# NVlabs/FoundationPose

Hardware: NVIDIA H100
Metric: pose-hypotheses/sec at 640x480 RGB-D, 252 hyp, 5 refine iters (higher is better)
Workload: dtype f16

## Files before the change

foundationpose_b200/csrc/fp_api.cu:

```cuda
#include <math.h>
#include <stdlib.h>
#include <string.h>

#include <algorithm>
#include <exception>
#include <map>
#include <memory>
#include <string>
#include <tuple>
#include <utility>
#include <vector>

#include "../../include/fpose.h"
#include "fp_attn.cuh"
#include "fp_common.cuh"
#include "fp_crop.cuh"
#include "fp_depth.cuh"
#include "fp_gemm.cuh"
#include "fp_vis.cuh"

namespace fp {
const char* get_last_error();

template <cudaError_t (*Free)(void*)>
// ... 74 lines not shown
struct MeshSlot {
  DevBuf vpos, vnrm, vatt, faces, meshlets, ml_verts, ml_tris, tex;
  int V = 0, F = 0, Ht = 0, Wt = 0, n_meshlets = 0, front_sign = 0, closed = 0;
  float bs[4] = {0.f, 0.f, 0.f, 0.f};
  bool has_tex = false, loaded = false;
  float diameter = 0.f;
};

struct CameraBufs {
  DevBuf rgb_raw, depth_raw, rgba, depth, xyz;
  PinnedBuf stage_rgb, stage_depth;
};

}

struct fp_ctx {
  int device = 0;
  fp::Net net[2];
  unsigned long long epoch = 1;
  unsigned long long graph_captures = 0;
  fp::MeshSlot mesh[fp::kMaxMeshes];
  fp::DevBuf mesh_table;
  float rot_normalizer = 0.3490658503988659f;
  float crop_ratio[2] = {1.2f, 1.2f};
  fp::CameraBufs cam[fp::kMaxCameras];
  fp::DevBuf depth_a;
  const float* depth_cur = nullptr;
  float K[9] = {0};
  int H = 0, W = 0;
  bool has_frame = false;
  int cap_n = 0;
  fp::DevBuf crops, act0, a1, a2, a3, ab0, ab1, ab2, c0, c1, c2, tok, qkv, att, x1pre, x1, ff, x2pre;
  fp::DevBuf head_out, poses_a, poses_b, feats, tail_qkv, tail_attn, tail_proj, scores, best;
  int tail_cap = 0;
  float fold_c = 0.f;
  fp::DevBuf fold_v, tail_counter;
  struct GraphEntry {
    cudaGraphExec_t exec = nullptr;
    unsigned long long epoch = 0;
    float K[9] = {0};
    int H = 0, W = 0;
  };
  std::map<std::tuple<int, int, int, int>, GraphEntry> graphs;
  std::map<std::tuple<int, int, int, int>, int> graph_nodes;
  cudaStream_t cap_stream = nullptr;
  cudaStream_t side_stream = nullptr;
  cudaEvent_t ev_fork = nullptr, ev_join = nullptr;
  int fork_max_n = 128;
  bool use_graphs = true;
  bool cull_backfaces = true;
  bool track_valid = false;
  int crop_tile = 0;
  fp::DevBuf lt_buf, lr_buf, feat_buf, pose_stage, tok_mean;
  fp::DevBuf mask_buf, mask_stats, crop_stats;
  fp::PinnedBuf stage_pose;
  fp::DevBuf track_pose;
  fp::PinnedBuf stage_poses;
  fp::DevBuf args;
  fp::PinnedBuf stage_args;
  int cam_grid_h = 0, cam_grid_w = 0;
  fp::DevBuf seg_off, reg_feats, mask_off;
  fp::PinnedBuf stage_masks, stage_ints;
  fp::DevBuf vis_rec, vis_range;
};

namespace fp {

static int ensure_capacity(fp_ctx* c, int N) {
  if (N <= c->cap_n) return 0;
  const size_t n = (size_t)N;
  int rc = 0;
  const size_t m = 2 * n + 3;
  rc |= dev_alloc(c->epoch, c->crops, m * kCropImg * 2, true);
  rc |= dev_alloc(c->epoch, c->act0, m * 80 * 80 * 64 * 2);
  rc |= dev_alloc(c->epoch, c->a1, m * 1600 * 128 * 2);
  rc |= dev_alloc(c->epoch, c->a2, m * 1600 * 128 * 2);
  rc |= dev_alloc(c->epoch, c->a3, m * 1600 * 128 * 2);
  rc |= dev_alloc(c->epoch, c->ab0, n * 1600 * 256 * 2);
  rc |= dev_alloc(c->epoch, c->ab1, n * 1600 * 256 * 2);
  rc |= dev_alloc(c->epoch, c->ab2, n * 1600 * 256 * 2);
  rc |= dev_alloc(c->epoch, c->c0, n * T * 512 * 2);
  rc |= dev_alloc(c->epoch, c->c1, n * T * 512 * 2);
  rc |= dev_alloc(c->epoch, c->c2, n * T * 512 * 2);
  rc |= dev_alloc(c->epoch, c->tok, n * T * 512 * 2);
  rc |= dev_alloc(c->epoch, c->qkv, n * T * 3072 * 2);
  rc |= dev_alloc(c->epoch, c->att, 2 * n * T * 512 * 2);
  rc |= dev_alloc(c->epoch, c->x1pre, 2 * n * T * 512 * 2);
  rc |= dev_alloc(c->epoch, c->x1, 2 * n * T * 512 * 2);
  rc |= dev_alloc(c->epoch, c->ff, 2 * n * T * 512 * 2);
  rc |= dev_alloc(c->epoch, c->x2pre, 2 * n * T * 512 * 2);
  rc |= dev_alloc(c->epoch, c->head_out, 2 * n * 3 * 4);
  rc |= dev_alloc(c->epoch, c->poses_a, n * 16 * 4);
  rc |= dev_alloc(c->epoch, c->poses_b, n * 16 * 4);
  rc |= dev_alloc(c->epoch, c->feats, n * 512 * 4);
  rc |= dev_alloc(c->epoch, c->lt_buf, n * 3 * 4);
  rc |= dev_alloc(c->epoch, c->lr_buf, n * 9 * 4);
  rc |= dev_alloc(c->epoch, c->feat_buf, n * 512 * 4);
  rc |= dev_alloc(c->epoch, c->pose_stage, n * 16 * 4);
  rc |= dev_alloc(c->epoch, c->tok_mean, n * 512 * 4);
  if (rc) return -2;
  c->cap_n = N;
  return 0;
}

static int ensure_tail(fp_ctx* c, int L) {
  if (L <= c->tail_cap) return 0;
  int rc = 0;
  rc |= dev_alloc(c->epoch, c->tail_qkv, (size_t)L * 1536 * 4);
  rc |= dev_alloc(c->epoch, c->tail_attn, (size_t)L * 512 * 4);
  rc |= dev_alloc(c->epoch, c->tail_proj, (size_t)L * 512 * 4);
  rc |= dev_alloc(c->epoch, c->scores, (size_t)L * 4);
  rc |= dev_alloc(c->epoch, c->best, 16);
  if (rc) return -2;
  c->tail_cap = L;
  return 0;
}

static GemmLayer mk(int kind, int n_img, int H, int W, int Cin, int Cout, const void* in, const __half* w,
                    const float* b, void* out, int relu, const void* res = nullptr, int out_ld = 0, int out_split = 0,
                    const float* post_add = nullptr) {
  GemmLayer L;
  L.kind = kind;
  L.n_img = n_img;
  L.Hin = H;
// ... 33 lines not shown
  FP_TRY(gemm_layer_launch(mk(LK_CONV3_S1, M, 40, 40, 128, 128, c->a2.p, W(5), B(5), c->ab0.p, 1, c->a3.p, 256, Np), st));
  FP_TRY(gemm_layer_launch(mk(LK_CONV3_S1, N, 40, 40, 256, 256, c->ab0.p, W(6), B(6), c->ab1.p, 1), st));
  FP_TRY(gemm_layer_launch(mk(LK_CONV3_S1, N, 40, 40, 256, 256, c->ab1.p, W(7), B(7), c->ab2.p, 1, c->ab0.p), st));
  FP_TRY(gemm_layer_launch(mk(LK_CONV3_S1, N, 40, 40, 256, 256, c->ab2.p, W(8), B(8), c->ab1.p, 1), st));
  FP_TRY(gemm_layer_launch(mk(LK_CONV3_S1, N, 40, 40, 256, 256, c->ab1.p, W(9), B(9), c->ab0.p, 1, c->ab2.p), st));
  FP_TRY(gemm_layer_launch(mk(LK_CONV3_S2, N, 40, 40, 256, 512, c->ab0.p, W(10), B(10), c->c0.p, 1), st));
  FP_TRY(gemm_layer_launch(mk(LK_CONV3_S1, N, 20, 20, 512, 512, c->c0.p, W(11), B(11), c->c1.p, 1), st));
  FP_TRY(gemm_layer_launch(mk(LK_CONV3_S1, N, 20, 20, 512, 512, c->c1.p, W(12), B(12), c->c2.p, 1, c->c0.p), st));
  FP_TRY(gemm_layer_launch(mk(LK_CONV3_S1, N, 20, 20, 512, 512, c->c2.p, W(13), B(13), c->c1.p, 1), st));
  FP_TRY(gemm_layer_launch(
      mk(LK_CONV3_S1, N, 20, 20, 512, 512, c->c1.p, W(14), B(14), c->tok.p, 1, c->c2.p, 0, 0, net.f("pe")), st));
  return 0;
}

static int run_refine_heads(fp_ctx* c, const Net& net, int N, cudaStream_t st) {
  const int M = N * T;
  FP_TRY(gemm_layer_launch(mk(LK_LINEAR, 1, 1, M, 512, 3072, c->tok.p, net.h("heads.in_w"), net.f("heads.in_b"), c->qkv.p, 0), st));
  AttnParams ap;
  ap.qkv = reinterpret_cast<const __half*>(c->qkv.p);
  ap.ld = 3072;
  ap.q_off = 0;
  ap.k_off = 512;
  ap.v_off = 1024;
  ap.group_col_stride = 1536;
  ap.n_groups = 2;
  ap.out = reinterpret_cast<__half*>(c->att.p);
  ap.ld_out = 512;
  ap.out_group_stride = (size_t)M * 512;
  ap.B = N;
  ap.T = T;
  ap.n_heads = 4;
  ap.scale = 0.08838834764831845f;
  FP_TRY(attn_core_launch(ap, st));
  const bool fork = N <= c->fork_max_n;
  if (fork) {
    if (!c->side_stream) {
      FP_CUDA_OK(cudaStreamCreateWithFlags(&c->side_stream, cudaStreamNonBlocking));
      FP_CUDA_OK(cudaEventCreateWithFlags(&c->ev_fork, cudaEventDisableTiming));
      FP_CUDA_OK(cudaEventCreateWithFlags(&c->ev_join, cudaEventDisableTiming));
    }
    FP_CUDA_OK(cudaEventRecord(c->ev_fork, st));
    FP_CUDA_OK(cudaStreamWaitEvent(c->side_stream, c->ev_fork, 0));
  }
  for (int g = 0; g < 2; ++g) {
    cudaStream_t sg = (fork && g == 1) ? c->side_stream : st;
    char nm[48];
    auto H = [&](const char* s) { snprintf(nm, sizeof nm, "head%d.%s", g, s); return net.h(nm); };
    auto Fp = [&](const char* s) { snprintf(nm, sizeof nm, "head%d.%s", g, s); return net.f(nm); };
    const size_t off = (size_t)g * M * 512;
    const __half* att_g = reinterpret_cast<const __half*>(c->att.p) + off;
    __half* x1pre = reinterpret_cast<__half*>(c->x1pre.p) + off;
    __half* x1 = reinterpret_cast<__half*>(c->x1.p) + off;
    __half* ff = reinterpret_cast<__half*>(c->ff.p) + off;
    __half* x2pre = reinterpret_cast<__half*>(c->x2pre.p) + off;
    const __half* w;
    const float* b;
    w = H("out_w"); b = Fp("out_b");
    if (fork && g == 1) pdl_skip_next();
    FP_TRY(gemm_layer_launch(mk(LK_LINEAR, 1, 1, M, 512, 512, att_g, w, b, x1pre, 0, c->tok.p), sg));
    const float* g1 = Fp("ln1_g");
    const float* b1 = Fp("ln1_b");
    FP_TRY(layernorm_launch(x1pre, x1, g1, b1, M, sg));
    w = H("ff1_w"); b = Fp("ff1_b");
    FP_TRY(gemm_layer_launch(mk(LK_LINEAR, 1, 1, M, 512, 512, x1, w, b, ff, 1), sg));
    w = H("ff2_w"); b = Fp("ff2_b");
    FP_TRY(gemm_layer_launch(mk(LK_LINEAR, 1, 1, M, 512, 512, ff, w, b, x2pre, 0, x1), sg));
    const float* g2 = Fp("ln2_g");
    const float* b2 = Fp("ln2_b");
    const float* fw = Fp("fin_w");
    const float* fb = Fp("fin_b");
    FP_TRY(head_final_launch(x2pre, g2, b2, fw, fb, reinterpret_cast<float*>(c->head_out.p) + (size_t)g * N * 3, N, T, 3, sg));
  }
  if (fork) {
    FP_CUDA_OK(cudaEventRecord(c->ev_join, c->side_stream));
    FP_CUDA_OK(cudaStreamWaitEvent(st, c->ev_join, 0));
    pdl_skip_next();
  }
  return 0;
}

static int run_score_feats(fp_ctx* c, const Net& net, int N, float* feats, cudaStream_t st) {
  const int M = N * T;
  FP_TRY(gemm_layer_launch(mk(LK_LINEAR, 1, 1, M, 512, 1536, c->tok.p, net.h("att.in_w"), net.f("att.in_b"), c->qkv.p, 0), st));
  AttnParams ap;
  ap.qkv = reinterpret_cast<const __half*>(c->qkv.p);
  ap.ld = 1536;
  ap.q_off = 0;
  ap.k_off = 512;
  ap.v_off = 1024;
  ap.group_col_stride = 0;
  ap.n_groups = 1;
// ... 515 lines not shown
#define FP_API_BEGIN try {
#define FP_API_END                                                        \
  }                                                                       \
  catch (const std::exception& e) {                                       \
    fp::set_last_error("%s: exception: %s", __func__, e.what());          \
    return -3;                                                            \
  }                                                                       \
  catch (...) {                                                           \
    fp::set_last_error("%s: unknown exception", __func__);                \
    return -3;                                                            \
  }

extern "C" {

int fp_create(fp_ctx** out) {
  FP_API_BEGIN
  if (!out) {
    set_last_error("fp_create: null output");
    return -1;
  }
  int dev = 0;
  FP_CUDA_OK(cudaGetDevice(&dev));
  cudaDeviceProp prop;
  FP_CUDA_OK(cudaGetDeviceProperties(&prop, dev));
  FP_REQUIRE(prop.major == 9 && prop.minor == 0, "libfpose targets sm_90a (H100); device %d is sm_%d%d", dev, prop.major,
             prop.minor);
  fp_ctx* c = new fp_ctx();
  c->device = dev;
  const char* ng = getenv("FPOSE_NO_GRAPH");
  c->use_graphs = !(ng && ng[0] == '1');
  const char* nc = getenv("FPOSE_NO_CULL");
  c->cull_backfaces = !(nc && nc[0] == '1');
  if (const char* fk = getenv("FPOSE_FORK_MAX_N")) c->fork_max_n = atoi(fk);
  *out = c;
  return 0;
  FP_API_END
}

int fp_destroy(fp_ctx* c) {
  FP_API_BEGIN
  if (!c) return 0;
  DeviceGuard dg(c->device);
  cudaDeviceSynchronize();
  for (auto& kv : c->graphs)
    if (kv.second.exec) cudaGraphExecDestroy(kv.second.exec);
  if (c->cap_stream) cudaStreamDestroy(c->cap_stream);
  if (c->side_stream) cudaStreamDestroy(c->side_stream);
  if (c->ev_fork) cudaEventDestroy(c->ev_fork);
  if (c->ev_join) cudaEventDestroy(c->ev_join);
  delete c;
  return 0;
  FP_API_END
}

int fp_set_config(fp_ctx* c, int which, float crop_ratio, float rot_normalizer) {
  FP_API_BEGIN
  FP_REQUIRE(c, "null ctx");
  FP_REQUIRE(which == 0 || which == 1, "fp_set_config: which must be 0 (refiner) or 1 (scorer)");
  FP_REQUIRE(crop_ratio > 0.f, "fp_set_config: crop_ratio must be positive");
  DeviceGuard dg(c->device);
  c->crop_ratio[which] = crop_ratio;
  if (which == 0) c->rot_normalizer = rot_normalizer;
  ++c->epoch;
  if (c->mesh_table.p) FP_TRY(write_mesh_table(c));
  return 0;
  FP_API_END
// ... 796 lines not shown
```

foundationpose_b200/csrc/fp_api_ops.cu:

```cuda
#include "../../include/fpose.h"
#include "fp_common.cuh"
#include "fp_attn.cuh"
#include "fp_crop.cuh"
#include "fp_gemm.cuh"

#include <vector>

namespace fp {
const char* get_last_error();
int prof_collect(int kind, double* total_ms, double* total_work, int* launches);
int pose_errors_launch(const float* pts, int P, const float* pred, int N, const float* gt, int n_gt, float* add_out,
                       float* adds_out, cudaStream_t stream);
int sym_pose_errors_launch(const float* pts, int P, const float* pred, int N, const float* gt, int n_gt, const float* sym,
                           int S, const float* K, int n_K, float* mssd_out, float* mspd_out, cudaStream_t stream);
}

static int check_device_ptr(const void* p, const char* what, const char* fn = "fp_pose_errors") {
  int dev = 0;
  FP_CUDA_OK(cudaGetDevice(&dev));
  cudaPointerAttributes a;
  const cudaError_t e = cudaPointerGetAttributes(&a, p);
  if (e != cudaSuccess) {
    cudaGetLastError();
    fp::set_last_error("%s: %s: cudaPointerGetAttributes failed (%s)", fn, what, cudaGetErrorString(e));
// ... 82 lines not shown
    info[5] = total;
    return 0;
  } catch (...) {
    fp::set_last_error("fp_op_build_meshlets: exception");
    return -3;
  }
}

int fp_op_attention(const void* qkv, void* out, int B, int impl, void* stream) {
  if (!qkv || !out) {
    fp::set_last_error("fp_op_attention: null argument");
    return -1;
  }
  fp::AttnParams ap;
  ap.qkv = reinterpret_cast<const __half*>(qkv);
  ap.ld = 1536;
  ap.q_off = 0;
  ap.k_off = 512;
  ap.v_off = 1024;
  ap.group_col_stride = 0;
  ap.n_groups = 1;
  ap.out = reinterpret_cast<__half*>(out);
  ap.ld_out = 512;
  ap.out_group_stride = 0;
  ap.B = B;
  ap.T = 400;
  ap.n_heads = 4;
  ap.scale = 0.08838834764831845f;
  cudaStream_t st = reinterpret_cast<cudaStream_t>(stream);
  (void)impl;
  return fp::attn_tc_launch(ap, st);
}

static fp::GemmLayer to_gemm_layer(const fp_gemm_layer_t* l) {
  fp::GemmLayer L;
  L.kind = l->kind;
  L.n_img = l->n_img;
  L.Hin = l->Hin;
  L.Win = l->Win;
  L.Cin = l->Cin;
  L.Cout = l->Cout;
  L.in = l->in;
  L.w = l->w;
  L.bias = l->bias;
  L.res = l->res;
  L.res_ld = l->res_ld;
  L.out = l->out;
  L.out_ld = l->out_ld;
  L.out_split = l->out_split;
  L.post_add = l->post_add;
  L.relu = l->relu;
  return L;
}

int fp_op_gemm_layer(const fp_gemm_layer_t* l, void* stream) {
  if (!l) {
    fp::set_last_error("fp_op_gemm_layer: null layer");
    return -1;
  }
  return fp::gemm_layer_launch(to_gemm_layer(l), reinterpret_cast<cudaStream_t>(stream));
}

int fp_op_gemm_tile_n(const fp_gemm_layer_t* l, int* tile_n) {
  if (!l || !tile_n) {
    fp::set_last_error("fp_op_gemm_tile_n: null argument");
    return -1;
// ... 39 lines not shown
```

foundationpose_b200/csrc/fp_attn.cuh:

```cuda
#pragma once
#include <cuda_fp16.h>
#include <cuda_runtime.h>
#include <stddef.h>

namespace fp {

struct AttnParams {
  const __half* qkv;
  int ld;
  int q_off, k_off, v_off;
  int group_col_stride;
  int n_groups;
  __half* out;
  int ld_out;
  size_t out_group_stride;
  int B, T, n_heads;
  float scale;
};
int attn_core_launch(const AttnParams& p, cudaStream_t stream);
int attn_tc_launch(const AttnParams& p, cudaStream_t stream);

int layernorm_launch(const __half* x, __half* y, const float* gamma, const float* beta, int rows, cudaStream_t stream);
int head_final_launch(const __half* x, const float* gamma, const float* beta, const float* w, const float* bias,
                      float* out, int B, int T, int out_dim, cudaStream_t stream);
int token_mean_proj_launch(const __half* x, const float* w_f32, const float* bias, float* mean_ws, float* out, int B, int T,
                           cudaStream_t stream);

struct ScoreTailParams {
  const float* feats;
  int L;
  const float* w_in;
  const float* b_in;
  const float* fold_v;
  float fold_c;
  float offset;
  float* qkv;
  float* scores;
  int* best;
  unsigned int* counter;
  const int* seg = nullptr;
  int n_seg = 1;
  int seg_max = 0;
};
int score_tail_launch(const ScoreTailParams& p, cudaStream_t stream);

struct MeshSlotDev;
int pose_update_launch(const float* pose_in, const float* trans, const float* rot, float* pose_out,
                       float* trans_delta_out, float* rot_delta_out, int N, const MeshSlotDev* slots, const int* mesh_of,
                       float trans_scale, float rot_normalizer, cudaStream_t stream);
int f32_to_f16_launch(const float* x, __half* y, size_t n, cudaStream_t stream);

}
```

foundationpose_b200/csrc/fp_common.cuh:

```cuda
#pragma once
#include <cuda.h>
#include <cuda_fp16.h>
#include <cuda_runtime.h>
#include <stdint.h>
#include <stdio.h>
#include <string.h>

#include <atomic>

namespace fp {

void note_launches(int n);
unsigned long long launch_count();
void set_capturing(bool on);
inline bool device_bit_test(const std::atomic<unsigned long long>& m) {
  int d = 0;
  cudaGetDevice(&d);
  return (m.load(std::memory_order_acquire) >> (d & 63)) & 1ull;
}
inline void device_bit_set(std::atomic<unsigned long long>& m) {
  int d = 0;
  cudaGetDevice(&d);
  m.fetch_or(1ull << (d & 63), std::memory_order_release);
}
// ... 76 lines not shown
      "mbarrier.try_wait.parity.shared::cta.b64 P1, [%0], %1, %2;\n\t"
      "@P1 bra DONE_%=;\n\t"
      "bra WAIT_%=;\n\t"
      "DONE_%=:\n\t"
      "}" ::"r"(smem_u32(bar)),
      "r"(parity), "r"(0x989680)
      : "memory");
}

__device__ __forceinline__ void tma_load_5d(const CUtensorMap* map, uint64_t* bar, void* dst,
                                            int c0, int c1, int c2, int c3, int c4) {
  asm volatile(
      "cp.async.bulk.tensor.5d.shared::cluster.global.mbarrier::complete_tx::bytes"
      " [%0], [%1, {%3, %4, %5, %6, %7}], [%2];" ::"r"(smem_u32(dst)),
      "l"(reinterpret_cast<uint64_t>(map)), "r"(smem_u32(bar)), "r"(c0), "r"(c1), "r"(c2),
      "r"(c3), "r"(c4)
      : "memory");
}
__device__ __forceinline__ void tma_load_2d(const CUtensorMap* map, uint64_t* bar, void* dst,
                                            int c0, int c1) {
  asm volatile(
      "cp.async.bulk.tensor.2d.shared::cluster.global.mbarrier::complete_tx::bytes"
      " [%0], [%1, {%3, %4}], [%2];" ::"r"(smem_u32(dst)),
      "l"(reinterpret_cast<uint64_t>(map)), "r"(smem_u32(bar)), "r"(c0), "r"(c1)
      : "memory");
}
__device__ __forceinline__ void tma_store_5d(const CUtensorMap* map, const void* src, int c0, int c1, int c2, int c3,
                                             int c4) {
  asm volatile("cp.async.bulk.tensor.5d.global.shared::cta.bulk_group [%0, {%2, %3, %4, %5, %6}], [%1];" ::"l"(
                   reinterpret_cast<uint64_t>(map)),
               "r"(smem_u32(src)), "r"(c0), "r"(c1), "r"(c2), "r"(c3), "r"(c4)
               : "memory");
}
__device__ __forceinline__ void tma_prefetch_desc(const CUtensorMap* map) {
  asm volatile("prefetch.tensormap [%0];" ::"l"(reinterpret_cast<uint64_t>(map)) : "memory");
}

__device__ __forceinline__ uint32_t cluster_nctarank() {
  uint32_t r;
  asm volatile("mov.u32 %0, %%cluster_nctarank;" : "=r"(r));
  return r;
}
__device__ __forceinline__ uint32_t cluster_ctarank() {
  uint32_t r;
  asm volatile("mov.u32 %0, %%cluster_ctarank;" : "=r"(r));
  return r;
}
__device__ __forceinline__ void cluster_sync_all() {
  asm volatile("barrier.cluster.arrive.release.aligned;" ::: "memory");
  asm volatile("barrier.cluster.wait.acquire.aligned;" ::: "memory");
}

template <uint32_t N>
__device__ __forceinline__ void regs_release() {
  asm volatile("setmaxnreg.dec.sync.aligned.u32 %0;" ::"n"(N));
}
template <uint32_t N>
__device__ __forceinline__ void regs_acquire() {
  asm volatile("setmaxnreg.inc.sync.aligned.u32 %0;" ::"n"(N));
}

__device__ __forceinline__ void wgmma_fence() { asm volatile("wgmma.fence.sync.aligned;" ::: "memory"); }
__device__ __forceinline__ void wgmma_commit() { asm volatile("wgmma.commit_group.sync.aligned;" ::: "memory"); }
template <int N>
__device__ __forceinline__ void wgmma_wait() {
  asm volatile("wgmma.wait_group.sync.aligned %0;" ::"n"(N) : "memory");
// ... 38 lines not shown
```

foundationpose_b200/ops.py:

```python
import ctypes as C

import torch

from . import _lib
from ._lib import lib


def _ptr(t):
    return None if t is None else C.c_void_p(t.data_ptr())


def _stream():
    return C.c_void_p(torch.cuda.current_stream().cuda_stream)


def _require_cuda(*ts):
    for t in ts:
        if t is not None and not t.is_cuda:
            raise _lib.FposeError("libfpose operators need CUDA tensors (there is no CPU path)")


def gemm_layer(kind, x, w_packed, bias, *, n_img, Hin, Win, Cin, Cout, out=None, out_ld=None, out_split=0,
               res=None, res_ld=0, post_add=None, relu=False):
    _require_cuda(x, w_packed, bias, res, post_add, out)
# ... 3 lines not shown
    elif kind == _lib.LAYER_CONV3_S1:
        Ho, Wo = Hin, Win
    else:
        Ho, Wo = Hin // 2, Win // 2
    if out is None:
        out_ld = Cout
        out = torch.empty(n_img, Ho, Wo, Cout, dtype=torch.float16, device=x.device)
    L = _lib.GemmLayer(kind, n_img, Hin, Win, Cin, Cout, _ptr(x), _ptr(w_packed), _ptr(bias), _ptr(res),
                       res_ld, _ptr(out), out_ld, out_split, _ptr(post_add), 1 if relu else 0)
    _lib.check(lib.fp_op_gemm_layer(C.byref(L), _stream()), "fp_op_gemm_layer")
    return out


def gemm_tile_n(kind, *, n_img, Hin, Win, Cin, Cout, out_split=0):
    lib.fp_op_gemm_tile_n.argtypes = [C.POINTER(_lib.GemmLayer), C.POINTER(C.c_int)]
    lib.fp_op_gemm_tile_n.restype = C.c_int
    L = _lib.GemmLayer(kind, n_img, Hin, Win, Cin, Cout, None, None, None, None, 0, None, Cout, out_split, None, 0)
    tile_n = C.c_int(0)
    _lib.check(lib.fp_op_gemm_tile_n(C.byref(L), C.byref(tile_n)), "fp_op_gemm_tile_n")
    return tile_n.value


lib.fp_op_attention.argtypes = [C.c_void_p, C.c_void_p, C.c_int, C.c_int, C.c_void_p]
lib.fp_op_attention.restype = C.c_int


def attention(qkv, impl=1):
    _require_cuda(qkv)
    assert qkv.dtype == torch.float16 and qkv.shape[1] == 1536 and qkv.shape[0] % 400 == 0
    B = qkv.shape[0] // 400
    out = torch.empty(qkv.shape[0], 512, dtype=torch.float16, device=qkv.device)
    _lib.check(lib.fp_op_attention(_ptr(qkv), _ptr(out), B, impl, _stream()), "fp_op_attention")
    return out
```

include/fpose.h:

```cpp
#ifndef FPOSE_H_
#define FPOSE_H_

#include <stddef.h>
#include <stdint.h>

#ifdef __cplusplus
extern "C" {
#endif

const char* fp_last_error(void);
unsigned long long fp_launch_count(void);

int fp_prof_enable(int on);
int fp_prof_collect(int kind, double* total_ms, double* total_work, int* launches);


#define FP_LAYER_LINEAR 0
#define FP_LAYER_CONV3_S1 1
#define FP_LAYER_CONV3_S2 2
#define FP_LAYER_CONV7_S2 3

typedef struct fp_gemm_layer {
  int kind;
  int n_img;
  int Hin, Win;
  int Cin;
  int Cout;
  const void* in;
  const void* w;
  const float* bias;
  const void* res;
  int res_ld;
  void* out;
  int out_ld;
  int out_split;
  const float* post_add;
  int relu;
} fp_gemm_layer_t;

int fp_op_gemm_layer(const fp_gemm_layer_t* layer, void* stream);
int fp_op_gemm_tile_n(const fp_gemm_layer_t* layer, int* tile_n);

int fp_op_attention(const void* qkv, void* out, int B, int impl, void* stream);



#define FP_METRICS_MAX_POINTS 131072
#define FP_METRICS_MAX_POSES (1 << 24)
int fp_pose_errors(const float* pts, int P, const float* pred, int N, const float* gt, int n_gt,
                   float* add_out, float* adds_out, void* stream);

#define FP_METRICS_MAX_SYMMETRIES 4096
int fp_sym_pose_errors(const float* pts, int P, const float* pred, int N, const float* gt, int n_gt, const float* sym,
                       int S, const float* K, int n_K, float* mssd_out, float* mspd_out, void* stream);

typedef struct fp_ctx fp_ctx;

int fp_create(fp_ctx** ctx);
int fp_destroy(fp_ctx* ctx);

int fp_set_config(fp_ctx* ctx, int which, float crop_ratio, float rot_normalizer);

typedef struct fp_tensor {
  const char* name;
  const void* data;
  int dtype;
  long long numel;
} fp_tensor_t;

int fp_load_network(fp_ctx* ctx, int which, const fp_tensor_t* tensors, int n);

int fp_set_mesh(fp_ctx* ctx, int V, int F, const float* pos, const float* nrm, const float* uv, const float* vcol,
                const int* faces, const unsigned char* tex_rgb, int Ht, int Wt, float diameter);
#define FP_MAX_MESHES 64
int fp_set_mesh_slot(fp_ctx* ctx, int slot, int V, int F, const float* pos, const float* nrm, const float* uv,
                     const float* vcol, const int* faces, const unsigned char* tex_rgb, int Ht, int Wt, float diameter);
// ... 81 lines not shown
```

Before: 3609.

## Fuse head out-proj/ff2 GEMMs with residual, LayerNorm and readout in full-row kernel

```diff
diff --git a/foundationpose_b200/csrc/fp_api.cu b/foundationpose_b200/csrc/fp_api.cu
--- a/foundationpose_b200/csrc/fp_api.cu
+++ b/foundationpose_b200/csrc/fp_api.cu
@@ -130,6 +130,7 @@
   int cap_n = 0;
   fp::DevBuf crops, act0, a1, a2, a3, ab0, ab1, ab2, c0, c1, c2, tok, qkv, att, x1pre, x1, ff, x2pre;
   fp::DevBuf head_out, poses_a, poses_b, feats, tail_qkv, tail_attn, tail_proj, scores, best;
+  fp::DevBuf head_tok;
   int tail_cap = 0;
   float fold_c = 0.f;
   fp::DevBuf fold_v, tail_counter;
@@ -144,6 +145,7 @@
   cudaStream_t cap_stream = nullptr;
   cudaStream_t side_stream = nullptr;
   cudaEvent_t ev_fork = nullptr, ev_join = nullptr;
+  bool fused_heads = true;
   int fork_max_n = 128;
   bool use_graphs = true;
   bool cull_backfaces = true;
@@ -188,6 +190,7 @@
   rc |= dev_alloc(c->epoch, c->ff, 2 * n * T * 512 * 2);
   rc |= dev_alloc(c->epoch, c->x2pre, 2 * n * T * 512 * 2);
   rc |= dev_alloc(c->epoch, c->head_out, 2 * n * 3 * 4);
+  rc |= dev_alloc(c->epoch, c->head_tok, 2 * n * T * 3 * 4);
   rc |= dev_alloc(c->epoch, c->poses_a, n * 16 * 4);
   rc |= dev_alloc(c->epoch, c->poses_b, n * 16 * 4);
   rc |= dev_alloc(c->epoch, c->feats, n * 512 * 4);
@@ -287,6 +290,7 @@
   ap.n_heads = 4;
   ap.scale = 0.08838834764831845f;
   FP_TRY(attn_core_launch(ap, st));
+  const bool fused = c->fused_heads;
   const bool fork = N <= c->fork_max_n;
   if (fork) {
     if (!c->side_stream) {
@@ -312,6 +316,32 @@
     const float* b;
     w = H("out_w"); b = Fp("out_b");
     if (fork && g == 1) pdl_skip_next();
+    if (fused) {
+      HeadLnArgs a;
+      a.M = M;
+      a.x = att_g;
+      a.w = w;
+      a.bias = b;
+      a.res = reinterpret_cast<const __half*>(c->tok.p);
+      a.gamma = Fp("ln1_g");
+      a.beta = Fp("ln1_b");
+      a.out = x1;
+      a.fin_w = nullptr;
+      a.tok_out = nullptr;
+      FP_TRY(head_ln1_launch(a, sg));
+      FP_TRY(gemm_layer_launch(mk(LK_LINEAR, 1, 1, M, 512, 512, x1, H("ff1_w"), Fp("ff1_b"), ff, 1), sg));
+      a.x = ff;
+      a.w = H("ff2_w");
+      a.bias = Fp("ff2_b");
+      a.res = x1;
+      a.gamma = Fp("ln2_g");
+      a.beta = Fp("ln2_b");
+      a.out = nullptr;
+      a.fin_w = Fp("fin_w");
+      a.tok_out = reinterpret_cast<float*>(c->head_tok.p) + (size_t)g * M * 3;
+      FP_TRY(head_readout_launch(a, Fp("fin_b"), reinterpret_cast<float*>(c->head_out.p) + (size_t)g * N * 3, N, T, sg));
+      continue;
+    }
     FP_TRY(gemm_layer_launch(mk(LK_LINEAR, 1, 1, M, 512, 512, att_g, w, b, x1pre, 0, c->tok.p), sg));
     const float* g1 = Fp("ln1_g");
     const float* b1 = Fp("ln1_b");
@@ -893,6 +923,8 @@
   const char* nc = getenv("FPOSE_NO_CULL");
   c->cull_backfaces = !(nc && nc[0] == '1');
   if (const char* fk = getenv("FPOSE_FORK_MAX_N")) c->fork_max_n = atoi(fk);
+  const char* fh = getenv("FPOSE_FUSED_HEADS");
+  c->fused_heads = !(fh && fh[0] == '0');
   *out = c;
   return 0;
   FP_API_END
diff --git a/foundationpose_b200/csrc/fp_api_ops.cu b/foundationpose_b200/csrc/fp_api_ops.cu
--- a/foundationpose_b200/csrc/fp_api_ops.cu
+++ b/foundationpose_b200/csrc/fp_api_ops.cu
@@ -138,6 +138,53 @@
   return fp::attn_tc_launch(ap, st);
 }
 
+static fp::HeadLnArgs head_args(int M, const void* x, const void* w, const float* bias, const void* res,
+                                const float* gamma, const float* beta) {
+  fp::HeadLnArgs a;
+  a.M = M;
+  a.x = reinterpret_cast<const __half*>(x);
+  a.w = reinterpret_cast<const __half*>(w);
+  a.bias = bias;
+  a.res = reinterpret_cast<const __half*>(res);
+  a.gamma = gamma;
+  a.beta = beta;
+  a.out = nullptr;
+  a.fin_w = nullptr;
+  a.tok_out = nullptr;
+  return a;
+}
+
+int fp_op_head_ln1(int M, const void* x, const void* w, const float* bias, const void* res, const float* gamma,
+                   const float* beta, void* out, void* stream) {
+  FP_REQUIRE(M > 0, "fp_op_head_ln1: M = %d", M);
+  fp::HeadLnArgs a = head_args(M, x, w, bias, res, gamma, beta);
+  a.out = reinterpret_cast<__half*>(out);
+  return fp::head_ln1_launch(a, reinterpret_cast<cudaStream_t>(stream));
+}
+
+int fp_op_head_readout(int N, int T, const void* x, const void* w, const float* bias, const void* res, const float* gamma,
+                       const float* beta, const float* fin_w, const float* fin_b, float* tok_ws, float* head_out,
+                       void* stream) {
+  FP_REQUIRE(N > 0 && T > 0, "fp_op_head_readout: N = %d, T = %d", N, T);
+  fp::HeadLnArgs a = head_args(N * T, x, w, bias, res, gamma, beta);
+  a.fin_w = fin_w;
+  a.tok_out = tok_ws;
+  return fp::head_readout_launch(a, fin_b, head_out, N, T, reinterpret_cast<cudaStream_t>(stream));
+}
+
+int fp_op_layernorm(const void* x, void* y, const float* gamma, const float* beta, int rows, void* stream) {
+  FP_REQUIRE(x && y && gamma && beta, "fp_op_layernorm: null argument");
+  return fp::layernorm_launch(reinterpret_cast<const __half*>(x), reinterpret_cast<__half*>(y), gamma, beta, rows,
+                              reinterpret_cast<cudaStream_t>(stream));
+}
+
+int fp_op_head_final(const void* x, const float* gamma, const float* beta, const float* fin_w, const float* fin_b,
+                     float* head_out, int N, int T, void* stream) {
+  FP_REQUIRE(x && gamma && beta && fin_w && fin_b && head_out, "fp_op_head_final: null argument");
+  return fp::head_final_launch(reinterpret_cast<const __half*>(x), gamma, beta, fin_w, fin_b, head_out, N, T, 3,
+                               reinterpret_cast<cudaStream_t>(stream));
+}
+
 static fp::GemmLayer to_gemm_layer(const fp_gemm_layer_t* l) {
   fp::GemmLayer L;
   L.kind = l->kind;
diff --git a/foundationpose_b200/csrc/fp_attn.cuh b/foundationpose_b200/csrc/fp_attn.cuh
--- a/foundationpose_b200/csrc/fp_attn.cuh
+++ b/foundationpose_b200/csrc/fp_attn.cuh
@@ -23,6 +23,21 @@
 int layernorm_launch(const __half* x, __half* y, const float* gamma, const float* beta, int rows, cudaStream_t stream);
 int head_final_launch(const __half* x, const float* gamma, const float* beta, const float* w, const float* bias,
                       float* out, int B, int T, int out_dim, cudaStream_t stream);
+struct HeadLnArgs {
+  int M;
+  const __half* x;
+  const __half* w;
+  const float* bias;
+  const __half* res;
+  const float* gamma;
+  const float* beta;
+  __half* out;
+  const float* fin_w;
+  float* tok_out;
+};
+int head_ln1_launch(const HeadLnArgs& a, cudaStream_t stream);
+int head_readout_launch(const HeadLnArgs& a, const float* fin_b, float* head_out, int N, int T, cudaStream_t stream);
+
 int token_mean_proj_launch(const __half* x, const float* w_f32, const float* bias, float* mean_ws, float* out, int B, int T,
                            cudaStream_t stream);
 
diff --git a/foundationpose_b200/csrc/fp_common.cuh b/foundationpose_b200/csrc/fp_common.cuh
--- a/foundationpose_b200/csrc/fp_common.cuh
+++ b/foundationpose_b200/csrc/fp_common.cuh
@@ -132,6 +132,12 @@
                "r"(smem_u32(src)), "r"(c0), "r"(c1), "r"(c2), "r"(c3), "r"(c4)
                : "memory");
 }
+__device__ __forceinline__ void tma_store_2d(const CUtensorMap* map, const void* src, int c0, int c1) {
+  asm volatile("cp.async.bulk.tensor.2d.global.shared::cta.bulk_group [%0, {%2, %3}], [%1];" ::"l"(
+                   reinterpret_cast<uint64_t>(map)),
+               "r"(smem_u32(src)), "r"(c0), "r"(c1)
+               : "memory");
+}
 __device__ __forceinline__ void tma_prefetch_desc(const CUtensorMap* map) {
   asm volatile("prefetch.tensormap [%0];" ::"l"(reinterpret_cast<uint64_t>(map)) : "memory");
 }
diff --git a/foundationpose_b200/csrc/fp_head.cu b/foundationpose_b200/csrc/fp_head.cu
--- /dev/null
+++ b/foundationpose_b200/csrc/fp_head.cu
@@ -0,0 +1,353 @@
+#include "fp_attn.cuh"
+#include "fp_common.cuh"
+#include "fp_gemm.cuh"
+#include "fp_wgmma.cuh"
+
+namespace fp {
+
+int encode_map_f16(CUtensorMap* map, const void* base, int rank, const uint64_t* dims, const uint64_t* strides_bytes,
+                   const uint32_t* box);
+
+#define FP_TRY_HEAD(expr) \
+  do {                    \
+    int _rc = (expr);     \
+    if (_rc) return _rc;  \
+  } while (0)
+
+constexpr int kHeadRows = 64;
+constexpr int kHeadC = 512;
+constexpr int kHeadNumKb = kHeadC / 64;
+constexpr int kHeadThreads = 384;
+constexpr int kHeadABytes = kHeadRows * 64 * 2;
+constexpr int kHeadWBoxBytes = 256 * 64 * 2;
+constexpr int kHeadStageBytes = kHeadABytes + 2 * kHeadWBoxBytes;
+constexpr int kHeadSlabBytes = kHeadRows * 64 * 2;
+constexpr int kHeadSlabs = kHeadC / 64;
+constexpr int kHeadStagingBytes = kHeadSlabs * kHeadSlabBytes;
+constexpr int kHeadRedBytes = 4096;
+constexpr int kHeadOut = 3;
+constexpr int kHeadPrmBytes = (3 + kHeadOut) * kHeadC * 4;
+constexpr int kHeadSmemOptIn = 232448;
+constexpr int kHeadStages = (kHeadSmemOptIn - kHeadStagingBytes - kHeadRedBytes - kHeadPrmBytes - 1024  -
+                             256 ) / kHeadStageBytes;
+constexpr int kHeadSmemBytes =
+    kHeadStages * kHeadStageBytes + kHeadStagingBytes + kHeadRedBytes + kHeadPrmBytes + 1024 + 256;
+static_assert(kHeadStages == 2, "the full-row head tile is planned for two 72 KB ring stages");
+static_assert(kHeadSmemBytes <= kHeadSmemOptIn, "head tile exceeds the 227 KB opt-in shared memory");
+constexpr int kHeadProducerRegs = 40;
+constexpr int kHeadConsumerRegs = 232;
+
+struct HeadLnParams {
+  int M, tiles;
+  const float* bias;
+  const float* gamma;
+  const float* beta;
+  const float* fin_w;
+  float* tok_out;
+  float eps;
+};
+
+template <bool kReadout>
+__global__ void __launch_bounds__(kHeadThreads, 1)
+    head_ln_kernel(const __grid_constant__ CUtensorMap map_a, const __grid_constant__ CUtensorMap map_w,
+                   const __grid_constant__ CUtensorMap map_res, const __grid_constant__ CUtensorMap map_out,
+                   const __grid_constant__ HeadLnParams p) {
+  constexpr int S = kHeadStages;
+  extern __shared__ uint8_t smem_raw[];
+  uint8_t* smem = smem_raw + ((1024u - (smem_u32(smem_raw) & 1023u)) & 1023u);
+  uint8_t* staging = smem + S * kHeadStageBytes;
+  float* red = reinterpret_cast<float*>(staging + kHeadStagingBytes);
+  float* red_sum = red;
+  float* red_sq = red + 128;
+  float* red_o = red + 256;
+  float* prm = reinterpret_cast<float*>(staging + kHeadStagingBytes + kHeadRedBytes);
+  float* bias_s = prm;
+  float* gamma_s = prm + kHeadC;
+  float* beta_s = prm + 2 * kHeadC;
+  float* finw_s = prm + 3 * kHeadC;
+  uint64_t* bars = reinterpret_cast<uint64_t*>(staging + kHeadStagingBytes + kHeadRedBytes + kHeadPrmBytes);
+  uint64_t* full = bars;
+  uint64_t* empty = bars + S;
+  uint64_t* res_full = bars + 2 * S;
+
+  if (threadIdx.x == 0) {
+    tma_prefetch_desc(&map_a);
+    tma_prefetch_desc(&map_w);
+    tma_prefetch_desc(&map_res);
+    if (!kReadout) tma_prefetch_desc(&map_out);
+    for (int s = 0; s < S; ++s) {
+      mbar_init(&full[s], 1);
+      mbar_init(&empty[s], 256);
+    }
+    mbar_init(res_full, 1);
+    mbar_fence_init();
+  }
+  __syncthreads();
+  pdl_trigger();
+  pdl_wait();
+
+  if (threadIdx.x < 128) {
+    regs_release<kHeadProducerRegs>();
+    if (threadIdx.x == 0) {
+      int stage = 0, phase = 0;
+      for (int t = blockIdx.x; t < p.tiles; t += gridDim.x) {
+        for (int kb = 0; kb < kHeadNumKb; ++kb) {
+          mbar_wait(&empty[stage], phase ^ 1);
+          uint8_t* sa = smem + stage * kHeadStageBytes;
+          mbar_expect_tx(&full[stage], kHeadStageBytes);
+          tma_load_2d(&map_a, &full[stage], sa, kb * 64, t * kHeadRows);
+          tma_load_2d(&map_w, &full[stage], sa + kHeadABytes, kb * 64, 0);
+          tma_load_2d(&map_w, &full[stage], sa + kHeadABytes + kHeadWBoxBytes, kb * 64, 256);
+          if (++stage == S) {
+            stage = 0;
+            phase ^= 1;
+          }
+        }
+      }
+    }
+    return;
+  }
+
+  regs_acquire<kHeadConsumerRegs>();
+  const int ct = threadIdx.x - 128;
+  const int cw = ct >> 7;
+  const int lane = threadIdx.x & 31;
+  const int r0 = 16 * ((ct >> 5) & 3) + (lane >> 2);
+  const int cq = 2 * (lane & 3);
+  const bool leader = (ct == 0);
+  const int col0 = 256 * cw + cq;
+  for (int i = ct; i < kHeadC; i += 256) {
+    bias_s[i] = p.bias[i];
+    gamma_s[i] = p.gamma[i];
+    beta_s[i] = p.beta[i];
+    if (kReadout)
+      for (int k = 0; k < kHeadOut; ++k) finw_s[k * kHeadC + i] = p.fin_w[k * kHeadC + i];
+  }
+  float acc[128];
+  int stage = 0, phase = 0, it = 0;
+  for (int t = blockIdx.x; t < p.tiles; t += gridDim.x, ++it) {
+    if (!kReadout && leader) asm volatile("cp.async.bulk.wait_group.read 0;" ::: "memory");
+    asm volatile("bar.sync 1, 256;" ::: "memory");
+    if (leader) {
+      mbar_expect_tx(res_full, kHeadStagingBytes);
+      for (int q = 0; q < kHeadSlabs; ++q) tma_load_2d(&map_res, res_full, staging + q * kHeadSlabBytes, 64 * q, t * kHeadRows);
+    }
+
+    int prev = -1;
+    for (int kb = 0; kb < kHeadNumKb; ++kb) {
+      mbar_wait(&full[stage], phase);
+      const uint32_t sa = smem_u32(smem + stage * kHeadStageBytes);
+      const uint64_t da = gmma_desc_sw128(sa);
+      const uint64_t db = gmma_desc_sw128(sa + kHeadABytes + (uint32_t)cw * kHeadWBoxBytes);
+      wgmma_fence();
+#pragma unroll
+      for (int k = 0; k < 4; ++k) Wgmma<256>::ss(acc, da + (uint64_t)(2 * k), db + (uint64_t)(2 * k), (kb > 0 || k > 0) ? 1u : 0u);
+      wgmma_commit();
+      if (prev >= 0) {
+        wgmma_wait<1>();
+        mbar_arrive(&empty[prev]);
+      }
+      prev = stage;
+      if (++stage == S) {
+        stage = 0;
+        phase ^= 1;
+      }
+    }
+    wgmma_wait<0>();
+    fence_regs(acc);
+    mbar_arrive(&empty[prev]);
+
+    mbar_wait(res_full, (uint32_t)(it & 1));
+    float rs[2] = {0.f, 0.f};
+#pragma unroll
+    for (int j = 0; j < 32; ++j) {
+      const float2 bb = *reinterpret_cast<const float2*>(bias_s + col0 + 8 * j);
+      const uint8_t* slab = staging + (4 * cw + (j >> 3)) * kHeadSlabBytes;
+#pragma unroll
+      for (int h = 0; h < 2; ++h) {
+        const int row = r0 + 8 * h;
+        const __half2 rh = *reinterpret_cast<const __half2*>(slab + row * 128 + (((uint32_t)(j & 7) ^ (uint32_t)(row & 7)) << 4) + cq * 2);
+        const float2 r = __half22float2(rh);
+        float a0 = acc[4 * j + 2 * h] + bb.x, a1 = acc[4 * j + 2 * h + 1] + bb.y;
+        a0 += r.x;
+        a1 += r.y;
+        const float2 v = __half22float2(__floats2half2_rn(a0, a1));
+        acc[4 * j + 2 * h] = v.x;
+        acc[4 * j + 2 * h + 1] = v.y;
+        rs[h] += v.x;
+        rs[h] += v.y;
+      }
+    }
+    float mean[2], rstd[2];
+#pragma unroll
+    for (int h = 0; h < 2; ++h) {
+      rs[h] += __shfl_xor_sync(0xffffffffu, rs[h], 1);
+      rs[h] += __shfl_xor_sync(0xffffffffu, rs[h], 2);
+      if ((lane & 3) == 0) red_sum[cw * 64 + r0 + 8 * h] = rs[h];
+    }
+    asm volatile("bar.sync 1, 256;" ::: "memory");
+    float qs[2] = {0.f, 0.f};
+#pragma unroll
+    for (int h = 0; h < 2; ++h) mean[h] = (red_sum[r0 + 8 * h] + red_sum[64 + r0 + 8 * h]) * (1.f / 512.f);
+#pragma unroll
+    for (int j = 0; j < 32; ++j)
+#pragma unroll
+      for (int h = 0; h < 2; ++h)
+#pragma unroll
+        for (int e = 0; e < 2; ++e) {
+          const float d = acc[4 * j + 2 * h + e] - mean[h];
+          qs[h] += d * d;
+        }
+#pragma unroll
+    for (int h = 0; h < 2; ++h) {
+      qs[h] += __shfl_xor_sync(0xffffffffu, qs[h], 1);
+      qs[h] += __shfl_xor_sync(0xffffffffu, qs[h], 2);
+      if ((lane & 3) == 0) red_sq[cw * 64 + r0 + 8 * h] = qs[h];
+    }
+    asm volatile("bar.sync 1, 256;" ::: "memory");
+#pragma unroll
+    for (int h = 0; h < 2; ++h)
+      rstd[h] = rsqrtf((red_sq[r0 + 8 * h] + red_sq[64 + r0 + 8 * h]) * (1.f / 512.f) + p.eps);
+
+    if constexpr (!kReadout) {
+#pragma unroll
+      for (int j = 0; j < 32; ++j) {
+        const float2 g = *reinterpret_cast<const float2*>(gamma_s + col0 + 8 * j);
+        const float2 b = *reinterpret_cast<const float2*>(beta_s + col0 + 8 * j);
+        uint8_t* slab = staging + (4 * cw + (j >> 3)) * kHeadSlabBytes;
+#pragma unroll
+        for (int h = 0; h < 2; ++h) {
+          const int row = r0 + 8 * h;
+          const float y0 = (acc[4 * j + 2 * h] - mean[h]) * rstd[h] * g.x + b.x;
+          const float y1 = (acc[4 * j + 2 * h + 1] - mean[h]) * rstd[h] * g.y + b.y;
+          *reinterpret_cast<uint32_t*>(slab + row * 128 + (((uint32_t)(j & 7) ^ (uint32_t)(row & 7)) << 4) + cq * 2) =
+              pack_half2(y0, y1);
+        }
+      }
+      asm volatile("fence.proxy.async.shared::cta;" ::: "memory");
+      asm volatile("bar.sync 1, 256;" ::: "memory");
+      if (leader) {
+        for (int q = 0; q < kHeadSlabs; ++q) tma_store_2d(&map_out, staging + q * kHeadSlabBytes, 64 * q, t * kHeadRows);
+        asm volatile("cp.async.bulk.commit_group;" ::: "memory");
+      }
+    } else {
+      float o[2][kHeadOut];
+#pragma unroll
+      for (int h = 0; h < 2; ++h)
+#pragma unroll
+        for (int k = 0; k < kHeadOut; ++k) o[h][k] = 0.f;
+#pragma unroll
+      for (int j = 0; j < 32; ++j) {
+        const float2 g = *reinterpret_cast<const float2*>(gamma_s + col0 + 8 * j);
+        const float2 b = *reinterpret_cast<const float2*>(beta_s + col0 + 8 * j);
+        float2 w[kHeadOut];
+#pragma unroll
+        for (int k = 0; k < kHeadOut; ++k) w[k] = *reinterpret_cast<const float2*>(finw_s + k * kHeadC + col0 + 8 * j);
+#pragma unroll
+        for (int h = 0; h < 2; ++h) {
+          const float y0 = (acc[4 * j + 2 * h] - mean[h]) * rstd[h] * g.x + b.x;
+          const float y1 = (acc[4 * j + 2 * h + 1] - mean[h]) * rstd[h] * g.y + b.y;
+#pragma unroll
+          for (int k = 0; k < kHeadOut; ++k) {
+            o[h][k] += y0 * w[k].x;
+            o[h][k] += y1 * w[k].y;
+          }
+        }
+      }
+#pragma unroll
+      for (int h = 0; h < 2; ++h)
+#pragma unroll
+        for (int k = 0; k < kHeadOut; ++k) {
+          o[h][k] += __shfl_xor_sync(0xffffffffu, o[h][k], 1);
+          o[h][k] += __shfl_xor_sync(0xffffffffu, o[h][k], 2);
+          if ((lane & 3) == 0) red_o[(cw * 64 + r0 + 8 * h) * kHeadOut + k] = o[h][k];
+        }
+      asm volatile("bar.sync 1, 256;" ::: "memory");
+      if (ct < 64 * kHeadOut) {
+        const int row = ct / kHeadOut, k = ct % kHeadOut;
+        const int m = t * kHeadRows + row;
+        if (m < p.M) p.tok_out[(size_t)m * kHeadOut + k] = red_o[row * kHeadOut + k] + red_o[(64 + row) * kHeadOut + k];
+      }
+    }
+  }
+  if (!kReadout && leader) asm volatile("cp.async.bulk.wait_group 0;" ::: "memory");
+}
+
+__global__ void __launch_bounds__(256) head_token_mean_kernel(const float* __restrict__ tok, const float* __restrict__ fin_b,
+                                                              float* __restrict__ out, int N, int T) {
+  pdl_trigger();
+  pdl_wait();
+  const int n = blockIdx.x * 8 + (threadIdx.x >> 5), lane = threadIdx.x & 31;
+  if (n >= N) return;
+  const float* x = tok + (size_t)n * T * kHeadOut;
+  float s[kHeadOut] = {0.f, 0.f, 0.f};
+  for (int t = lane; t < T; t += 32)
+#pragma unroll
+    for (int k = 0; k < kHeadOut; ++k) s[k] += x[t * kHeadOut + k];
+#pragma unroll
+  for (int k = 0; k < kHeadOut; ++k) {
+#pragma unroll
+    for (int o = 16; o > 0; o >>= 1) s[k] += __shfl_xor_sync(0xffffffffu, s[k], o);
+  }
+  if (lane < kHeadOut) {
+    const float v = lane == 0 ? s[0] : (lane == 1 ? s[1] : s[2]);
+    out[n * kHeadOut + lane] = v / (float)T + fin_b[lane];
+  }
+}
+
+template <bool kReadout>
+static int head_ln_launch(const HeadLnArgs& a, cudaStream_t stream) {
+  if (a.M == 0) return 0;
+  FP_REQUIRE(a.M > 0 && a.x && a.w && a.bias && a.res && a.gamma && a.beta, "head_ln: missing argument");
+  FP_REQUIRE(kReadout ? (a.fin_w && a.tok_out) : (a.out != nullptr), "head_ln: missing output");
+  static std::atomic<unsigned long long> attr_mask{0};
+  if (!device_bit_test(attr_mask)) {
+    FP_CUDA_OK(cudaFuncSetAttribute(head_ln_kernel<kReadout>, cudaFuncAttributeMaxDynamicSharedMemorySize, kHeadSmemBytes));
+    device_bit_set(attr_mask);
+  }
+  const uint64_t dims[2] = {(uint64_t)kHeadC, (uint64_t)a.M};
+  const uint64_t str[1] = {(uint64_t)kHeadC * 2};
+  const uint32_t box[2] = {64, (uint32_t)kHeadRows};
+  const uint64_t wdims[2] = {(uint64_t)kHeadC, (uint64_t)kHeadC};
+  const uint32_t wbox[2] = {64, 256};
+  CUtensorMap ma, mw, mr, mo;
+  FP_TRY_HEAD(encode_map_f16(&ma, a.x, 2, dims, str, box));
+  FP_TRY_HEAD(encode_map_f16(&mw, a.w, 2, wdims, str, wbox));
+  FP_TRY_HEAD(encode_map_f16(&mr, a.res, 2, dims, str, box));
+  if (kReadout) mo = mr;
+  else FP_TRY_HEAD(encode_map_f16(&mo, a.out, 2, dims, str, box));
+  HeadLnParams p;
+  p.M = a.M;
+  p.tiles = (a.M + kHeadRows - 1) / kHeadRows;
+  p.bias = a.bias;
+  p.gamma = a.gamma;
+  p.beta = a.beta;
+  p.fin_w = a.fin_w;
+  p.tok_out = a.tok_out;
+  p.eps = 1e-5f;
+  const int sms = num_sms();
+  FP_REQUIRE(sms > 0, "no CUDA device");
+  const int grid = p.tiles < sms ? p.tiles : sms;
+  prof_mark_begin(0, 2.0 * a.M * kHeadC * kHeadC, stream);
+  FP_CUDA_OK(launch_pdl(head_ln_kernel<kReadout>, dim3(grid), dim3(kHeadThreads), kHeadSmemBytes, stream, 1, ma, mw, mr, mo, p));
+  prof_mark_end(stream);
+  note_launches(1);
+  FP_CUDA_OK(cudaGetLastError());
+  return 0;
+}
+
+int head_ln1_launch(const HeadLnArgs& a, cudaStream_t stream) { return head_ln_launch<false>(a, stream); }
+
+int head_readout_launch(const HeadLnArgs& a, const float* fin_b, float* head_out, int N, int T, cudaStream_t stream) {
+  FP_REQUIRE(a.M == N * T, "head_readout: M = %d is not N * T = %d * %d", a.M, N, T);
+  FP_REQUIRE(fin_b && head_out, "head_readout: missing fin_b / head_out");
+  if (N == 0) return 0;
+  FP_TRY_HEAD(head_ln_launch<true>(a, stream));
+  FP_CUDA_OK(launch_pdl(head_token_mean_kernel, dim3((N + 7) / 8), dim3(256), 0, stream, 1, (const float*)a.tok_out, fin_b,
+                        head_out, N, T));
+  note_launches(1);
+  FP_CUDA_OK(cudaGetLastError());
+  return 0;
+}
+
+}
diff --git a/foundationpose_b200/ops.py b/foundationpose_b200/ops.py
--- a/foundationpose_b200/ops.py
+++ b/foundationpose_b200/ops.py
@@ -59,3 +59,60 @@
     out = torch.empty(qkv.shape[0], 512, dtype=torch.float16, device=qkv.device)
     _lib.check(lib.fp_op_attention(_ptr(qkv), _ptr(out), B, impl, _stream()), "fp_op_attention")
     return out
+
+
+_f = C.c_void_p
+lib.fp_op_head_ln1.argtypes = [C.c_int, _f, _f, _f, _f, _f, _f, _f, _f]
+lib.fp_op_head_ln1.restype = C.c_int
+lib.fp_op_head_readout.argtypes = [C.c_int, C.c_int, _f, _f, _f, _f, _f, _f, _f, _f, _f, _f, _f]
+lib.fp_op_head_readout.restype = C.c_int
+lib.fp_op_layernorm.argtypes = [_f, _f, _f, _f, C.c_int, _f]
+lib.fp_op_layernorm.restype = C.c_int
+lib.fp_op_head_final.argtypes = [_f, _f, _f, _f, _f, _f, C.c_int, C.c_int, _f]
+lib.fp_op_head_final.restype = C.c_int
+
+
+def _head_inputs(x, w, bias, res, gamma, beta):
+    _require_cuda(x, w, bias, res, gamma, beta)
+    assert x.dtype == w.dtype == res.dtype == torch.float16 and bias.dtype == gamma.dtype == beta.dtype == torch.float32
+    assert x.shape[-1] == 512 and w.shape == (512, 512) and res.shape == x.shape
+    return x.contiguous(), w.contiguous(), res.contiguous()
+
+
+def head_ln1(x, w, bias, res, gamma, beta):
+    x, w, res = _head_inputs(x, w, bias, res, gamma, beta)
+    out = torch.empty_like(x)
+    _lib.check(lib.fp_op_head_ln1(x.shape[0], _ptr(x), _ptr(w), _ptr(bias), _ptr(res), _ptr(gamma), _ptr(beta), _ptr(out),
+                                  _stream()), "fp_op_head_ln1")
+    return out
+
+
+def head_readout(x, w, bias, res, gamma, beta, fin_w, fin_b, T=400):
+    x, w, res = _head_inputs(x, w, bias, res, gamma, beta)
+    _require_cuda(fin_w, fin_b)
+    assert x.shape[0] % T == 0 and fin_w.shape == (3, 512) and fin_w.dtype == torch.float32
+    N = x.shape[0] // T
+    tok = torch.empty(x.shape[0], 3, dtype=torch.float32, device=x.device)
+    out = torch.empty(N, 3, dtype=torch.float32, device=x.device)
+    _lib.check(lib.fp_op_head_readout(N, T, _ptr(x), _ptr(w), _ptr(bias), _ptr(res), _ptr(gamma), _ptr(beta),
+                                      _ptr(fin_w.contiguous()), _ptr(fin_b), _ptr(tok), _ptr(out), _stream()),
+               "fp_op_head_readout")
+    return out, tok
+
+
+def layernorm(x, gamma, beta):
+    _require_cuda(x, gamma, beta)
+    x = x.contiguous()
+    y = torch.empty_like(x)
+    _lib.check(lib.fp_op_layernorm(_ptr(x), _ptr(y), _ptr(gamma), _ptr(beta), x.shape[0], _stream()), "fp_op_layernorm")
+    return y
+
+
+def head_final(x, gamma, beta, fin_w, fin_b, T=400):
+    _require_cuda(x, gamma, beta, fin_w, fin_b)
+    x = x.contiguous()
+    N = x.shape[0] // T
+    out = torch.empty(N, 3, dtype=torch.float32, device=x.device)
+    _lib.check(lib.fp_op_head_final(_ptr(x), _ptr(gamma), _ptr(beta), _ptr(fin_w.contiguous()), _ptr(fin_b), _ptr(out), N, T,
+                                    _stream()), "fp_op_head_final")
+    return out
diff --git a/include/fpose.h b/include/fpose.h
--- a/include/fpose.h
+++ b/include/fpose.h
@@ -42,6 +42,15 @@
 int fp_op_gemm_tile_n(const fp_gemm_layer_t* layer, int* tile_n);
 
 int fp_op_attention(const void* qkv, void* out, int B, int impl, void* stream);
+
+int fp_op_head_ln1(int M, const void* x, const void* w, const float* bias, const void* res, const float* gamma,
+                   const float* beta, void* out, void* stream);
+int fp_op_head_readout(int N, int T, const void* x, const void* w, const float* bias, const void* res, const float* gamma,
+                       const float* beta, const float* fin_w, const float* fin_b, float* tok_ws, float* head_out,
+                       void* stream);
+int fp_op_layernorm(const void* x, void* y, const float* gamma, const float* beta, int rows, void* stream);
+int fp_op_head_final(const void* x, const float* gamma, const float* beta, const float* fin_w, const float* fin_b,
+                     float* head_out, int N, int T, void* stream);
 
 
 
```

After: 3710, median of 6. +2.8%, better.
